# mFinn27/Template-Matching-and-Regression-MapReduce

Measured on AMD Instinct MI355X. Metric: images/sec (whole node) match+regress+NMS; % HBM/MFMA roofline at 1/2/4/8 GPU, higher is better.
Workload: dtype fp32; 1 GPU; config B: 64x SAM feats 256x64x64 (->128x128), 3 exemplars, templates 3x3-15x15, fp32, cls 0.1, IoU 0.5; config=B, images_per_gpu=64, exemplars=3, parallelism=dp1, decoder=split, decoder_precision=fp32

## Files before the change

### template-matching-and-regression-mapreduce_amd/csrc/conv_split.hip

```cpp
#include <algorithm>
#include <type_traits>

#include "tmr_common.h"

namespace {

typedef _Float16 h8 __attribute__((ext_vector_type(8)));
typedef __bf16 b8 __attribute__((ext_vector_type(8)));
typedef float f32x4 __attribute__((ext_vector_type(4)));
typedef __bf16 b4 __attribute__((ext_vector_type(4)));
typedef __attribute__((address_space(3))) void *lds_ptr_t;


constexpr int BM = 128;
constexpr int TH = 16;
constexpr int TW = 32;
constexpr int LDS_KB = 160;
constexpr int PXG = 8, NG = 4;
constexpr int NWAVES = 8;
constexpr int NTHREADS = NWAVES * 64;
constexpr int WNS = (NWAVES == 8 || TH == 8) ? 2 : 1;
static_assert(TH == 4 * NWAVES / WNS, "a wave owns 4 output rows");
constexpr int NIN = 8 / WNS;
constexpr int ACCW = NIN * 8 * 64 * 4;
// ... 332 lines not shown
                }
        }
    } else {
#pragma unroll
        for (int in = 0; in < NIN; ++in)
#pragma unroll
            for (int jp = 0; jp < 8; ++jp)
#pragma unroll
                for (int r = 0; r < 4; ++r) acc[in][jp][r] = 0.0f;
    }

    const int aoff = kg * WPL + (wn * 64 + l16) * 16;
    const int boff = kg * HPL + (wpix * 4 * HC + l16) * 16;

    auto ipt_of = [](bool lo_) { return lo_ ? 8 : G::NPLW * 2; };
#pragma unroll
    for (int m = 0; m < MPW; ++m) halo_dma1(0, m);
#pragma unroll
    for (int g0 = 0; g0 < D; ++g0) {
        const bool lo0 = HALVES == 2 && ((g0 / SPC) & 1);
        const int nt0 = min(TPS, T - (g0 % SPC) * TPS) * ipt_of(lo0) / NWAVES;
#pragma unroll
        for (int m = 0; m < nt0; ++m) w_dma1(g0, ipt_of(lo0), m);
    }
    asm volatile("s_waitcnt vmcnt(0)" ::: "memory");
    __builtin_amdgcn_s_barrier();
    for (int c = 0; c < NC; ++c) {
        auto half_chunk = [&](auto part_c) {
            constexpr int part = decltype(part_c)::value;
            constexpr bool lo = part == 1;
            const int hc = c * HALVES + part;
            const char *hl = Hs + (hc & 1) * HB;
            auto step = [&](auto sg_c) {
                constexpr int sg = decltype(sg_c)::value;
                constexpr bool L3 = G::LO3;
                constexpr int TPSx = L3 ? G::tps(part) : TPS;
                const int g = L3 ? c * G::SPCC + (part ? SPC : 0) + sg : hc * SPC + sg;
                constexpr bool lastx = sg + 1 >= G::spc(part);
                constexpr int pn = lastx ? 1 - part : part, sgn = lastx ? 0 : sg + 1;
                constexpr int nh = L3 ? G::nhp(part, sg) : G::nh(sg);
                constexpr bool loD = L3 ? pn == 1 : G::lo_of(sg + D, part, HALVES);
                constexpr int nw = L3 ? G::ntapp(pn, sgn) * G::ipt(pn == 1) / NWAVES : G::nw(sg, part, HALVES);
                constexpr int NSLOT = nh + nw;
                auto dma_slot = [&](int k) {
                    if constexpr (L3) {
                        if (k < nh)
                            halo_dma1(hc + 1, sg * G::qh(part) + k);
                        else
                            w_dma3(lastx && part == 1 ? c + 1 : c, pn, sgn, ipt_of(loD), k - nh);
                    } else {
                        if (k < nh)
                            halo_dma1(hc + 1, sg * Q + k);
                        else
                            w_dma1(g + D, ipt_of(loD), k - nh);
                    }
                };
                const char *wl = Ws + (g % NWB) * WB;
                constexpr int NA = (HALVES == 2 && !lo) ? 2 * NIN : NIN;
                constexpr int DB = NA >= 8 ? 1 : 2;
                constexpr int APG = NA >= 8 ? NA / 8 : 1;
                constexpr int NB = DB + 1;
                constexpr int ntap = L3 ? G::ntapp(part, sg) : (T - sg * TPS < TPS ? T - sg * TPS : TPS);
                constexpr int WB1x = L3 ? G::wb1(part) : WB1;
                auto afrag = [&](int tl, int i) -> V {
                    return *reinterpret_cast<const V *>(wl + tl * WB1x + (i / NIN) * 4 * WPL + aoff +
                                                        (i % NIN) * 256);
                };
                auto bfrag = [&](int tap, int jp) -> V {
                    const int ky = tap / KS, kx = tap % KS;
                    return *reinterpret_cast<const V *>(
                        hl + boff + (((jp >> 1) + ky) * HC + kx + (jp & 1) * 16) * 16);
                };
                V aw[2][NA];
                V bx[NB];
#pragma unroll
                for (int i = 0; i < NA; ++i) aw[0][i] = afrag(0, i);
#pragma unroll
                for (int d = 0; d < DB; ++d) bx[d] = bfrag(sg * TPSx, d);
                __builtin_amdgcn_sched_group_barrier(0x100, NA + DB, 0);
#pragma unroll
                for (int tl = 0; tl < TPSx; ++tl) {
                    if (tl >= ntap) break;
                    const int tap = sg * TPSx + tl;
                    const bool more = tl + 1 < ntap;
#pragma unroll
                    for (int jp = 0; jp < 8; ++jp) {
                        const int q = tl * 8 + jp, qn = q + DB;
                        const bool rb = jp + DB < 8 || more;
                        if (rb) bx[qn % NB] = jp + DB < 8 ? bfrag(tap, jp + DB) : bfrag(tap + 1, jp + DB - 8);
                        const int na = (more && jp * APG < NA) ? APG : 0;
#pragma unroll
                        for (int j = 0; j < APG; ++j)
                            if (j < na) aw[(tl + 1) & 1][jp * APG + j] = afrag(tl + 1, jp * APG + j);
                        const int k = q - 1;
                        const bool dm = k >= 0 && k < NSLOT;
                        if (dm) dma_slot(k);
                        const V b = bx[q % NB];
#pragma unroll
                        for (int i = 0; i < NA; ++i)
                            acc[i % NIN][jp] = mma(aw[tl & 1][i], b, acc[i % NIN][jp]);
                        const int nr = (rb ? 1 : 0) + na;
                        if (nr == 3)
                            __builtin_amdgcn_sched_group_barrier(0x100, 3, 0);
                        else if (nr == 2)
                            __builtin_amdgcn_sched_group_barrier(0x100, 2, 0);
                        else if (nr == 1)
                            __builtin_amdgcn_sched_group_barrier(0x100, 1, 0);
                        if (dm) __builtin_amdgcn_sched_group_barrier(0x020, 1, 0);
                        __builtin_amdgcn_sched_group_barrier(0x008, NA, 0);
                    }
                }
#pragma unroll
                for (int k = 0; k < 16; ++k)
                    if (k >= ntap * 8 - 1 && k < NSLOT) dma_slot(k);
                __builtin_amdgcn_sched_barrier(0);
                if constexpr (D == 1)
                    asm volatile("s_waitcnt vmcnt(0)" ::: "memory");
                else
                    wait_vmcnt(G::allowed(sg, part, HALVES));
                __builtin_amdgcn_s_barrier();
            };
            [&]<int... SG>(std::integer_sequence<int, SG...>) {
                (step(std::integral_constant<int, SG>{}), ...);
            }(std::make_integer_sequence<int, G::LO3 ? G::spc(part) : SPC>{});
        };
        half_chunk(std::integral_constant<int, 0>{});
        if constexpr (HALVES == 2) half_chunk(std::integral_constant<int, 1>{});
    }
    asm volatile("s_waitcnt vmcnt(0)" ::: "memory");

    const float inv = 1.0f / sxw;
    if (EPI == 0 && (a.flags & TMR_SPLIT_TILED_OUT) && (a.flags & TMR_SPLIT_OUT_BF16)) {
        b4 *o = reinterpret_cast<b4 *>(a.out) + ((((size_t)u * a.NT + nt) * a.MT + mt) * NWAVES + wave) * ACCW / 4 +
                lane;
#pragma unroll
        for (int in = 0; in < NIN; ++in)
#pragma unroll
            for (int jp = 0; jp < 8; ++jp)
                __builtin_nontemporal_store(__builtin_convertvector(acc[in][jp] * inv, b4), o + (in * 8 + jp) * 64);
        return;
    }
    if (EPI == 0 && (a.flags & TMR_SPLIT_TILED_OUT)) {
        f32x4 *o = reinterpret_cast<f32x4 *>(
                       a.out + ((((size_t)u * a.NT + nt) * a.MT + mt) * NWAVES + wave) * ACCW) +
                   lane;
#pragma unroll
        for (int in = 0; in < NIN; ++in)
#pragma unroll
            for (int jp = 0; jp < 8; ++jp) {
                __builtin_nontemporal_store(acc[in][jp] * inv, o + (in * 8 + jp) * 64);
            }
        return;
    }
    float *red = reinterpret_cast<float *>(lds);
    float *sb = red + 4 * 8 * NHEAD * 16;
    float *shw = sb + BM;
    if (tid < BM) {
        const int n = nt * BM + tid;
        sb[tid] = n < a.N ? a.bias[n] : 0.0f;
    }
    if (EPI == 1)
        for (int e = tid; e < BM * NHEAD; e += NTHREADS) shw[e] = a.headw[(size_t)nt * BM * NHEAD + e];
    __syncthreads();
    if constexpr (EPI == 0) {
        float invp[8];
#pragma unroll
        for (int jp = 0; jp < 8; ++jp) {
            invp[jp] = inv;
            const int y = ty0 + wpix * 4 + (jp >> 1), x = tx0 + (jp & 1) * 16 + l16;
            if (PR::SCALED && (a.flags & TMR_SPLIT_XMAX_PER_PIXEL) && y < a.H && x < a.W)
                invp[jp] = 1.0f / (split_scale(a.xmax + ((size_t)u * a.H + y) * a.W + x) * split_scale(a.wmax));
        }
#pragma unroll
        for (int in = 0; in < NIN; ++in)
#pragma unroll
            for (int r = 0; r < 4; ++r) {
                const int nl = wn * 64 + in * 16 + 4 * kg + r;
                const int n = nt * BM + nl;
                const bool nin = n < a.N;
                const float bn = sb[nl];
#pragma unroll
                for (int jp = 0; jp < 8; ++jp) {
                    const int y = ty0 + wpix * 4 + (jp >> 1), x = tx0 + (jp & 1) * 16 + l16;
                    float v = acc[in][jp][r] * invp[jp] + bn;
                    if (a.leaky) v = v >= 0.0f ? v : v * 0.01f;
                    if (nin && y < a.H && x < a.W) a.out[((size_t)u * a.N + n) * HW + (size_t)y * a.W + x] = v;
                }
            }
        return;
    }
    f2 hs2[4][NHEAD];
#pragma unroll
    for (int q = 0; q < 4; ++q)
#pragma unroll
        for (int k = 0; k < NHEAD; ++k) hs2[q][k] = (f2){0.0f, 0.0f};
    const f2 inv2 = {inv, inv};
#pragma unroll
    for (int in = 0; in < NIN; ++in)
#pragma unroll
        for (int r = 0; r < 4; ++r) {
            const int nl = wn * 64 + in * 16 + 4 * kg + r;
            const f2 bn2 = {sb[nl], sb[nl]};
            f2 hw2[NHEAD];
#pragma unroll
            for (int k = 0; k < NHEAD; ++k) hw2[k] = (f2){shw[nl * NHEAD + k], shw[nl * NHEAD + k]};
#pragma unroll
            for (int q = 0; q < 4; ++q)
                head_fma(head_act((f2){acc[in][2 * q][r], acc[in][2 * q + 1][r]}, inv2, bn2, a.leaky), hw2, hs2[q]);
            __builtin_amdgcn_sched_barrier(0);
        }
    float X[40];
#pragma unroll
    for (int q = 0; q < 4; ++q)
#pragma unroll
        for (int k = 0; k < NHEAD; ++k) {
            X[2 * (5 * q + k)] = hs2[q][k].x;
            X[2 * (5 * q + k) + 1] = hs2[q][k].y;
        }
    float Y[20], Z[10];
#pragma unroll
    for (int m = 0; m < 20; ++m) {
        const auto s = __builtin_amdgcn_permlane16_swap(__float_as_uint(X[2 * m]), __float_as_uint(X[2 * m + 1]),
                                                         false, false);
        Y[m] = __uint_as_float(s[0]) + __uint_as_float(s[1]);
    }
#pragma unroll
    for (int p = 0; p < 10; ++p) {
        const auto s = __builtin_amdgcn_permlane32_swap(__float_as_uint(Y[2 * p]), __float_as_uint(Y[2 * p + 1]),
                                                         false, false);
        Z[p] = __uint_as_float(s[0]) + __uint_as_float(s[1]);
    }
    __syncthreads();
    if (WNS == 2 && wn == 1) {
#pragma unroll
        for (int p = 0; p < 10; ++p) red[((wpix * 10 + p) * 4 + kg) * 16 + l16] = Z[p];
    }
    __syncthreads();
    if (wn == 0) {
#pragma unroll
        for (int p = 0; p < 10; ++p) {
            const int j = 4 * p + kg, m = j >> 1, q = m / NHEAD, k = m - q * NHEAD;
            const int jp = 2 * q + (j & 1);
            const int y = ty0 + wpix * 4 + (jp >> 1), x = tx0 + (jp & 1) * 16 + l16;
            const float v = Z[p] + (WNS == 2 ? red[((wpix * 10 + p) * 4 + kg) * 16 + l16] : 0.0f);
            if (y < a.H && x < a.W) a.partials[(((size_t)nt * NHEAD + k) * a.U + u) * HW + (size_t)y * a.W + x] = v;
        }
    }
}

template <int KS, int PREC, int EPI>
int launch_split(SArgs a, hipStream_t s) {
    constexpr size_t lds = Geo<KS, PREC>::LDS;
    static_assert(lds <= 160 * 1024, "LDS");
    static_assert((4 * 8 * NHEAD * 16 + BM * (NHEAD + 1)) * 4 <= lds, "epilogue scratch");
    auto kern = split_conv_kernel<KS, PREC, EPI>;
    if (tmr_set_max_lds((const void *)kern, lds) !=
        hipSuccess)
        return TMR_E_HIP;
    const int64_t blocks = (int64_t)a.NTW * a.MT * a.U;
    if (blocks <= 0) return TMR_OK;
    TMR_REQUIRE(blocks < (1ll << 31));
    hipLaunchKernelGGL(kern, dim3((unsigned)blocks), dim3(NTHREADS), lds, s, a);
    TMR_CHECK_LAUNCH();
    return TMR_OK;
}

template <int KS, int EPI>
int dispatch_prec(int prec, const SArgs &a, hipStream_t s) {
    switch (prec) {
        case TMR_PREC_F16X3: return launch_split<KS, TMR_PREC_F16X3, EPI>(a, s);
        case TMR_PREC_BF16: return launch_split<KS, TMR_PREC_BF16, EPI>(a, s);
        case TMR_PREC_F16: return launch_split<KS, TMR_PREC_F16, EPI>(a, s);
        default: return TMR_E_INVALID;
    }
}

template <int EPI>
int dispatch_ks(int ks, int prec, const SArgs &a, hipStream_t s) {
    switch (ks) {
        case 1: return dispatch_prec<1, EPI>(prec, a, s);
        case 3: return dispatch_prec<3, EPI>(prec, a, s);
        case 5: return dispatch_prec<5, EPI>(prec, a, s);
        case 7: return dispatch_prec<7, EPI>(prec, a, s);
        default: return TMR_E_INVALID;
    }
}

constexpr int PT = TMR_POINTS_TILE;
constexpr int PP = 2 * PT;
constexpr int PCG = PP / 16;
constexpr int PTW = NWAVES / WNS;
static_assert(PT == 64 && 4 * PP == NTHREADS, "points block: one store lane per head and point");
static_assert(WNS == 2 && NWAVES == 2 * P, "points block: a wave per 64-channel half; gathers dealt by (piece, half)");

struct PArgs {
    SArgs s;
    const float *head_bias;
    const float *box;
    const int32_t *tiles;
    int ntiles;
    float *b;
};

template <int KS, int PREC>
__global__ __launch_bounds__(NTHREADS) void split_points_kernel(PArgs pa) {
    typedef Prec<PREC> PR;
    typedef typename PR::V V;
    constexpr int T = KS * KS, HALVES = PR::HALVES, WREC = PR::WREC;
    constexpr int NF = NIN;
    constexpr int NS = HALVES == 2 ? 3 * T : T;
    const SArgs &a = pa.s;
    constexpr int BB = T * P * PP * 16;
    extern __shared__ __attribute__((aligned(16))) char plds[];
    char *Bs = plds;
    float(*red)[4][PP] = reinterpret_cast<float(*)[4][PP]>(plds + 2 * BB);
    float(*xch)[4][PP] = reinterpret_cast<float(*)[4][PP]>(plds + BB);
    static_assert(PTW * 4 * PP * sizeof(float) <= BB, "the odd waves' sums fit a B buffer");

    const int tid = threadIdx.x;
    const int lane = tid & 63;
    const int wave = __builtin_amdgcn_readfirstlane(tid >> 6);
    const int wh = wave & 1, wt = wave >> 1;
    const int l16 = lane & 15, kg = lane >> 4;
    const int HW = a.H * a.W;
    int tu[2], tfirst[2], tcnt[2], timg[2];
    float sxw[2];
#pragma unroll
    for (int hh = 0; hh < 2; ++hh) {
        const int64_t ti = 2 * (int64_t)blockIdx.x + hh;
        const bool have = ti < pa.ntiles;
        const int32_t *tl = pa.tiles + 3 * (have ? ti : ti - hh);
        tu[hh] = min(max(tl[0], 0), a.U - 1);
        tfirst[hh] = min(max(tl[1], 0), HW - 1);
        tcnt[hh] = have ? min(max(tl[2], 0), PT) : 0;
        timg[hh] = a.unit_image ? a.unit_image[tu[hh]] : tu[hh];
        sxw[hh] = split_sxw<PREC>(a, tu[hh]);
    }
    const int NC = a.NC0 + a.NC1;
    auto pixel = [&](int u, int first, int cnt, int p) {
        const int *pixi = reinterpret_cast<const int *>(pa.box) + 4 * (size_t)u * HW;
        return min(max(pixi[4 * (size_t)min(first + (p < cnt ? p : 0), HW - 1)], 0), HW - 1);
    };
    const int gu = wh ? tu[1] : tu[0], gfirst = wh ? tfirst[1] : tfirst[0], gcnt = wh ? tcnt[1] : tcnt[0];
    const int gimg = wh ? timg[1] : timg[0];

    const uint32_t cstride = (uint32_t)a.Hp * a.Wp * XREC;
    const int h0 = a.NC0 * HALVES, h1 = a.NC1 * HALVES;
    const __amdgpu_buffer_rsrc_t xr0 = __builtin_amdgcn_make_buffer_rsrc(
        (void *)(h0 ? a.x0 + (size_t)gimg * h0 * cstride : a.x1), (short)0, h0 * cstride, 0x00020000);
    const __amdgpu_buffer_rsrc_t xr1 = __builtin_amdgcn_make_buffer_rsrc(
        (void *)(h1 ? a.x1 + (size_t)gu * h1 * cstride : a.x0), (short)0, h1 * cstride, 0x00020000);
    const uint32_t tapstride = (uint32_t)NC * a.Npad * WREC;
    const __amdgpu_buffer_rsrc_t wr = __builtin_amdgcn_make_buffer_rsrc(
        (void *)a.wp, (short)0, T * tapstride, 0x00020000);
    uint32_t goff[KS];
#pragma unroll
    for (int i = 0; i < KS; ++i) {
        const int g = 64 * i + lane;
        const int pix = pixel(gu, gfirst, gcnt, g / KS), y = pix / a.W;
        goff[i] = (uint32_t)(y * a.Wp + (pix - y * a.W) + g % KS) * 16;
    }
    const uint32_t qstride = (uint32_t)a.Hp * a.Wp * 16;
    auto gather = [&](int hc) {
        const bool s0 = hc < h0;
        const uint32_t hs_ = (uint32_t)(s0 ? hc : hc - h0) * cstride + wt * qstride;
#pragma unroll
        for (int ky = 0; ky < KS; ++ky)
#pragma unroll
            for (int i = 0; i < KS; ++i)
                buffer_lds16(s0 ? xr0 : xr1,
                             (lds_ptr_t)(Bs + (hc & 1) * BB + (((ky * P + wt) * PP + wh * PT) * KS + 64 * i) * 16), goff[i],
                             hs_ + (uint32_t)(ky * a.Wp) * 16);
    };
    const int bfo = kg * (PP * KS * 16) + l16 * (KS * 16);
    auto bfrag = [&](int hc, int tap, int j) -> V {
        return *reinterpret_cast<const V *>(Bs + (hc & 1) * BB + (tap / KS) * (P * PP * KS * 16) + bfo +
                                            j * (16 * KS * 16) + (tap % KS) * 16);
    };

    const int npass = a.NTW > PTW ? 2 : 1;
    for (int pass = 0; pass < npass; ++pass) {
        const int wtile = pass * PTW + wt;
        const bool active = wtile < a.NTW;
        const int nt = a.NT0 + (active ? wtile : 0);
        const uint32_t aoff = (uint32_t)kg * a.Npad * 16 + ((uint32_t)nt * BM + wh * (BM / 2) + l16) * 16;
        gather(0);

        f32x4 acc[NF][PCG];
        if (a.acc_init) {
            const bool i16 = a.flags & TMR_SPLIT_INIT_BF16;
#pragma unroll
            for (int j = 0; j < PCG; ++j) {
                constexpr int HJ = PCG / 2;
                const int hh = j / HJ;
                const int pix = pixel(tu[hh], tfirst[hh], tcnt[hh], (j % HJ) * 16 + l16);
                const int py = pix / a.W, px = pix - py * a.W;
                const float sx = sxw[hh];
                const int islab = (a.flags & TMR_SPLIT_INIT_BCAST) ? 0 : timg[hh];
                const int mt = (py / TH) * a.TXN + px / TW;
                const int wpix = (py % TH) >> 2, jp = ((py & 3) << 1) | ((px % TW) >> 4);
                const size_t g4 = (((((size_t)islab * a.NT + nt) * a.MT + mt) * NWAVES + wpix * WNS + wh) * ACCW) / 4 +
                                  jp * 64 + kg * 16 + (px & 15);
                if (i16) {
                    const b4 *ai = reinterpret_cast<const b4 *>(a.acc_init) + g4;
#pragma unroll
                    for (int f = 0; f < NF; ++f)
                        acc[f][j] = __builtin_convertvector(ai[f * 8 * 64], f32x4) * sx;
                } else {
                    const f32x4 *ai = reinterpret_cast<const f32x4 *>(a.acc_init) + g4;
#pragma unroll
                    for (int f = 0; f < NF; ++f)
                        acc[f][j] = ai[f * 8 * 64] * sx;
                }
            }
        } else {
#pragma unroll
            for (int f = 0; f < NF; ++f)
#pragma unroll
                for (int j = 0; j < PCG; ++j) acc[f][j] = (f32x4){0.0f, 0.0f, 0.0f, 0.0f};
        }

        auto st_part = [](int s) { return HALVES == 2 && s >= 2 * T ? 1 : 0; };
        auto st_tap = [](int s) { return HALVES == 2 ? (s >= 2 * T ? s - 2 * T : s / 2) : s; };
        auto st_term = [](int s) { return HALVES == 2 && s < 2 * T ? s & 1 : 0; };
        auto st_newb = [](int s) { return !(HALVES == 2 && s < 2 * T && (s & 1)); };
        auto st_first = [](int s) { return s == 0 || (HALVES == 2 && s == 2 * T); };
        auto st_last = [](int s) { return s == NS - 1 || (HALVES == 2 && s == 2 * T - 1); };
        constexpr int AR = 3;
        static_assert(NS % AR == 0 && NS >= AR, "weight ring");
        V ar[AR][NF];
        auto load_stage = [&](int c, int s) {
            if (s >= NS) {
                s -= NS;
                c = c + 1 < NC ? c + 1 : c;
            }
            const uint32_t as = (uint32_t)st_tap(s) * tapstride + (uint32_t)c * a.Npad * WREC +
                                (uint32_t)st_term(s) * 4 * a.Npad * 16;
#pragma unroll
            for (int f = 0; f < NF; ++f) ar[s % AR][f] = buffer_load16<V>(wr, aoff + f * 256, as);
        };
#pragma unroll
        for (int s = 0; s < AR - 1; ++s) load_stage(0, s);
        asm volatile("s_waitcnt vmcnt(0)" ::: "memory");
        __syncthreads();
        V bc[PCG];
        const int NHC = NC * HALVES;
        for (int c = 0; c < NC; ++c) {
#pragma unroll
            for (int s = 0; s < NS; ++s) {
                const int hc = c * HALVES + st_part(s);
                load_stage(c, s + AR - 1);
                if (st_first(s)) {
                    if (hc + 1 < NHC) gather(hc + 1);
#pragma unroll
                    for (int j = 0; j < PCG; ++j) bc[j] = bfrag(hc, st_tap(s), j);
                }
                const bool nextb = s + 1 < NS && st_newb(s + 1) && !st_first(s + 1);
                __builtin_amdgcn_sched_barrier(0);
#pragma unroll
                for (int j = 0; j < PCG; ++j) {
#pragma unroll
                    for (int f = 0; f < NF; ++f) acc[f][j] = mma(ar[s % AR][f], bc[j], acc[f][j]);
                    if (nextb) {
                        bc[j] = bfrag(hc, st_tap(s + 1), j);
                        __builtin_amdgcn_sched_barrier(0);
                    }
                }
                __builtin_amdgcn_sched_barrier(0);
                if (st_last(s)) {
                    static_assert((AR - 1) * NF == 8 && T > AR - 1, "the counted wait below");
                    asm volatile("s_waitcnt vmcnt(8)" ::: "memory");
                    __syncthreads();
                }
            }
        }

        f2 hs[PCG / 2][NHEAD];
#pragma unroll
        for (int q = 0; q < PCG / 2; ++q)
#pragma unroll
            for (int k = 0; k < NHEAD; ++k) hs[q][k] = (f2){0.0f, 0.0f};
#pragma unroll
        for (int f = 0; f < NF; ++f)
#pragma unroll
            for (int r = 0; r < 4; ++r) {
                const int n = nt * BM + wh * (BM / 2) + f * 16 + 4 * kg + r;
                const float bv = n < a.N ? a.bias[n] : 0.0f;
                const f2 bn2 = {bv, bv};
                f2 hw2[NHEAD];
#pragma unroll
                for (int k = 0; k < NHEAD; ++k) {
                    const float h = a.headw[(size_t)n * NHEAD + k];
                    hw2[k] = (f2){h, h};
                }
#pragma unroll
                for (int q = 0; q < PCG / 2; ++q) {
                    const float inv = 1.0f / sxw[q / (PCG / 4)];
                    head_fma(head_act((f2){acc[f][2 * q][r], acc[f][2 * q + 1][r]}, (f2){inv, inv}, bn2, a.leaky), hw2,
                             hs[q]);
                }
            }
        float z[PCG / 2][4][2];
#pragma unroll
        for (int q = 0; q < PCG / 2; ++q)
#pragma unroll
            for (int k = 0; k < 4; ++k)
#pragma unroll
                for (int e = 0; e < 2; ++e) {
                    const float x = hs[q][k][e];
                    const float y = x + __shfl_xor(x, 16);
                    z[q][k][e] = y + __shfl_xor(y, 32);
                }
        if (wh == 1 && kg == 0 && active) {
#pragma unroll
            for (int q = 0; q < PCG / 2; ++q)
#pragma unroll
                for (int k = 0; k < 4; ++k)
#pragma unroll
                    for (int e = 0; e < 2; ++e) xch[wt][k][(2 * q + e) * 16 + l16] = z[q][k][e];
        }
        __syncthreads();
        if (wh == 0 && kg == 0 && active) {
#pragma unroll
            for (int q = 0; q < PCG / 2; ++q)
#pragma unroll
                for (int k = 0; k < 4; ++k)
#pragma unroll
                    for (int e = 0; e < 2; ++e) {
                        const int p = (2 * q + e) * 16 + l16;
                        red[wtile][k][p] = z[q][k][e] + xch[wt][k][p];
                    }
        }
    }
    __syncthreads();
    {
        const int k = tid / PP, p = tid % PP, pl = p % PT;
        if (pl < gcnt) {
            const int pix = pixel(gu, gfirst, gcnt, pl);
            float s = 0.0f;
            for (int t = 0; t < a.NTW; ++t) s += red[t][k][p];
            pa.b[((size_t)gu * 4 + k) * HW + pix] = s + pa.head_bias[k];
        }
    }
}

template <int PREC>
int launch_points(const PArgs &pa, int ntiles, hipStream_t s) {
    constexpr size_t lds = 2 * 9 * P * PP * 16 + NWAVES * 4 * PP * sizeof(float);
    static_assert(lds <= LDS_KB * 1024, "LDS");
    auto kern = split_points_kernel<3, PREC>;
    if (tmr_set_max_lds((const void *)kern, lds) != hipSuccess) return TMR_E_HIP;
    hipLaunchKernelGGL(kern, dim3((unsigned)((ntiles + 1) / 2)), dim3(NTHREADS), lds, s, pa);
    TMR_CHECK_LAUNCH();
    return TMR_OK;
}

inline int prec_halves(int prec) { return prec == TMR_PREC_F16X3 ? 2 : 1; }
inline int prec_wrec(int prec) { return prec == TMR_PREC_F16X3 ? 128 : 64; }
inline bool prec_ok(int prec) {
    return prec == TMR_PREC_F16X3 || prec == TMR_PREC_BF16 || prec == TMR_PREC_F16;
}
inline bool ks_ok(int ks) { return ks == 1 || ks == 3 || ks == 5 || ks == 7; }
inline bool tile_window(int flags, int NT, int &first, int &count) {
    first = (flags >> TMR_SPLIT_TILE_FIRST_SHIFT) & 0xff;
    count = (flags >> TMR_SPLIT_TILE_COUNT_SHIFT) & 0x7f;
    if (count == 0) {
        if (first != 0) return false;
        count = NT;
    }
    return first + count <= NT;
}
inline int pad_h(int H, int ks) { return (int)tmr_cdiv(H, TH) * TH + ks - 1; }
inline int pad_w(int W, int ks) { return (int)tmr_cdiv(W, TW) * TW + ks - 1; }

__device__ __forceinline__ void absmax_commit(float m, unsigned *out) {
    __shared__ float red[4];
    for (int o = 32; o > 0; o >>= 1) m = fmaxf(m, __shfl_xor(m, o));
    if ((threadIdx.x & 63) == 0) red[threadIdx.x >> 6] = m;
    __syncthreads();
    if (threadIdx.x == 0) atomicMax(out, __float_as_uint(fmaxf(fmaxf(red[0], red[1]), fmaxf(red[2], red[3]))));
}

__global__ __launch_bounds__(256) void absmax_rows_kernel(const float *__restrict__ x, int64_t n, int vec,
                                                          unsigned *__restrict__ out) {
    const float *xr = x + (size_t)blockIdx.y * n;
    float m = 0.0f;
    const int64_t step = (int64_t)gridDim.x * blockDim.x;
    if (vec) {
        const float4 *x4 = reinterpret_cast<const float4 *>(xr);
        for (int64_t i = (int64_t)blockIdx.x * blockDim.x + threadIdx.x; i < n / 4; i += step) {
            const float4 v = x4[i];
            m = fmaxf(m, fmaxf(fmaxf(fabsf(v.x), fabsf(v.y)), fmaxf(fabsf(v.z), fabsf(v.w))));
        }
    } else {
        for (int64_t i = (int64_t)blockIdx.x * blockDim.x + threadIdx.x; i < n; i += step)
            m = fmaxf(m, fabsf(xr[i]));
    }
    absmax_commit(m, out + blockIdx.y);
}

constexpr int PA_PIX = 64, PA_GRP = 8;
__global__ __launch_bounds__(PA_PIX * PA_GRP) void pixel_absmax_kernel(const float *__restrict__ x, int S, int C,
                                                                       int64_t HW, float *__restrict__ out) {
    __shared__ float part[PA_GRP][PA_PIX];
    const int lane = threadIdx.x & (PA_PIX - 1), grp = threadIdx.x / PA_PIX;
    const int64_t i = (int64_t)blockIdx.x * PA_PIX + lane;
    float m = 0.0f;
    if (i < (int64_t)S * HW) {
        const int64_t s = i / HW, p = i - s * HW;
        const float *xp = x + (size_t)s * C * HW + p;
#pragma unroll 8
        for (int c = grp; c < C; c += PA_GRP) m = fmaxf(m, fabsf(xp[(size_t)c * HW]));
    }
    part[grp][lane] = m;
    __syncthreads();
    if (grp == 0 && i < (int64_t)S * HW) {
#pragma unroll
        for (int g = 1; g < PA_GRP; ++g) m = fmaxf(m, part[g][lane]);
        out[i] = m;
    }
}

__global__ __launch_bounds__(256) void scale_merge_kernel(const float *__restrict__ img_max,
                                                          const float *__restrict__ unit_max,
                                                          const int32_t *__restrict__ unit_image, int U,
                                                          float *__restrict__ out_img,
                                                          float *__restrict__ out_unit) {
    __shared__ float red[4];
    const int b = blockIdx.x;
    float m = 0.0f;
    for (int u = threadIdx.x; u < U; u += blockDim.x)
        if (unit_image[u] == b) m = fmaxf(m, unit_max[u]);
    for (int o = 32; o > 0; o >>= 1) m = fmaxf(m, __shfl_xor(m, o));
    if ((threadIdx.x & 63) == 0) red[threadIdx.x >> 6] = m;
    __syncthreads();
    m = fmaxf(fmaxf(red[0], red[1]), fmaxf(red[2], red[3]));
    if (img_max) m = fmaxf(m, img_max[b]);
    if (threadIdx.x == 0 && out_img) out_img[b] = m;
    for (int u = threadIdx.x; u < U; u += blockDim.x)
        if (unit_image[u] == b) out_unit[u] = m;
}

template <int PREC, int MODE>
__global__ void xpack_kernel(const float *__restrict__ x, int S, int Cin, int Hin, int Win, int ups,
                             int ones, int H, int W, int NCc, int Hp, int Wp, int pad,
                             const float *__restrict__ xmax, int xms,
                             typename Prec<PREC>::V *__restrict__ out) {
    constexpr int HALVES = Prec<PREC>::HALVES;
    const int64_t total = (int64_t)S * NCc * Hp * Wp;
    const int64_t i = (int64_t)blockIdx.x * blockDim.x + threadIdx.x;
    if (i >= total) return;
    const int xp = (int)(i % Wp);
    int64_t r = i / Wp;
    const int yp = (int)(r % Hp);
    r /= Hp;
    const int c = (int)(r % NCc);
    const int s = (int)(r / NCc);
    const int y = yp - pad, xx = xp - pad;
    const bool in = y >= 0 && y < H && xx >= 0 && xx < W;
    const float *xm = !xmax ? nullptr
                      : xms == 2 ? (in ? xmax + ((size_t)s * H + y) * W + xx : nullptr)
                                 : xmax + (size_t)s * xms;
    const float sc = Prec<PREC>::SCALED ? split_scale(xm) : 1.0f;
    float v[CCH];
#pragma unroll
    for (int k = 0; k < CCH; ++k) {
        const int ch = c * CCH + k;
        float val = 0.0f;
        if (in) {
            if (MODE == 0) {
                if (ch < Cin) val = x[(((size_t)s * Cin + ch) * H + y) * W + xx];
            } else if (ch < Cin) {
                const float *pl = x + ((size_t)s * Cin + ch) * Hin * Win;
                val = ups ? up_value(pl, Hin, Win, y, xx) : pl[(size_t)y * Win + xx];
            } else if (ones && ch == Cin) {
                val = 1.0f;
            }
        }
        v[k] = val;
    }
    typename Prec<PREC>::V hi[P], lo[P];
    split_record<PREC>(v, sc, hi, lo);
    const size_t plane = (size_t)Hp * Wp;
    typename Prec<PREC>::V *o = out + ((size_t)s * NCc + c) * HALVES * P * plane + (size_t)yp * Wp + xp;
#pragma unroll
    for (int q = 0; q < P; ++q) o[q * plane] = hi[q];
    if (HALVES == 2) {
#pragma unroll
        for (int q = 0; q < P; ++q) o[(P + q) * plane] = lo[q];
    }
}

constexpr int XSEG = 128;
constexpr int XPACK16_RPB = 4;
template <int PREC, typename IN = float, int RPB = 1>
__global__ __launch_bounds__(256) void xpack4_kernel(const IN *__restrict__ x, int S, int Cin, int H, int W,
                                                     int NCc, int Hp, int Wp, int pad, int64_t nseg,
                                                     int64_t nbord, const float *__restrict__ xmax, int xms,
                                                     typename Prec<PREC>::V *__restrict__ out) {
    constexpr int HALVES = Prec<PREC>::HALVES;
    typedef typename Prec<PREC>::V V;
    typedef typename Prec<PREC>::E E;
    constexpr int VE = 16 / sizeof(IN);
    constexpr int LPR = CCH * XSEG / VE;
    typedef IN INV __attribute__((ext_vector_type(VE)));
    static_assert(RPB * LPR % 256 == 0 && RPB * XSEG * P % 256 == 0 && XSEG % VE == 0, "xpack4 tiling");
    __shared__ __attribute__((aligned(16))) IN tile[RPB][CCH][XSEG];
    const size_t plane = (size_t)Hp * Wp;
    const int t = threadIdx.x;
    if ((int64_t)blockIdx.x < nseg) {
        const int nsx = (W + XSEG - 1) / XSEG, nyg = (H + RPB - 1) / RPB;
        int64_t r = blockIdx.x;
        const int sx = (int)(r % nsx);
        r /= nsx;
        const int y0 = (int)(r % nyg) * RPB;
        r /= nyg;
        const int c = (int)(r % NCc);
        const int s = (int)(r / NCc);
        const int x0 = sx * XSEG, nx = min(XSEG, W - x0);
        const IN *src = x + ((size_t)s * Cin + (size_t)c * CCH) * H * W + (size_t)y0 * W + x0;
#pragma unroll
        for (int k = 0; k < RPB * LPR / 256; ++k) {
            const int e = t + 256 * k, rr = e / LPR, ch = (e % LPR) / (XSEG / VE), xv = e % (XSEG / VE);
            INV v = {};
            if (VE * xv < nx && c * CCH + ch < Cin && y0 + rr < H)
                v = *reinterpret_cast<const INV *>(src + (size_t)ch * H * W + (size_t)rr * W + VE * xv);
            *reinterpret_cast<INV *>(&tile[rr][ch][VE * xv]) = v;
        }
        __syncthreads();
        const float sc = Prec<PREC>::SCALED ? split_scale(xmax ? xmax + (size_t)s * xms : nullptr) : 1.0f;
        V *o = out + ((size_t)s * NCc + c) * HALVES * P * plane + (size_t)(y0 + pad) * Wp + x0 + pad;
#pragma unroll
        for (int k = 0; k < RPB * XSEG * P / 256; ++k) {
            const int e = t + 256 * k, rr = e / (XSEG * P), q = (e % (XSEG * P)) / XSEG, px = e % XSEG;
            if (px < nx && y0 + rr < H) {
                V hi, lo;
#pragma unroll
                for (int m = 0; m < 8; ++m) {
                    const float xs = (float)tile[rr][q * 8 + m][px] * sc;
                    const E h = (E)xs;
                    hi[m] = h;
                    if (HALVES == 2) lo[m] = (E)(xs - (float)h);
                }
                o[q * plane + (size_t)rr * Wp + px] = hi;
                if (HALVES == 2) o[(P + q) * plane + (size_t)rr * Wp + px] = lo;
            }
        }
        return;
    }
    const int64_t b0 = ((int64_t)blockIdx.x - nseg) * 256 + t;
    if (b0 >= nbord * S * NCc) return;
    const int64_t sc_i = b0 / nbord;
    int64_t b = b0 - sc_i * nbord;
    const int64_t top = (int64_t)pad * Wp, bot = (int64_t)(Hp - H - pad) * Wp;
    int yp, xp;
    if (b < top) {
        yp = (int)(b / Wp), xp = (int)(b % Wp);
    } else if ((b -= top) < bot) {
        yp = H + pad + (int)(b / Wp), xp = (int)(b % Wp);
    } else {
        b -= bot;
        const int side = Wp - W, k = (int)(b % side);
        yp = pad + (int)(b / side), xp = k < pad ? k : W + k;
    }
    V *o = out + (size_t)sc_i * HALVES * P * plane + (size_t)yp * Wp + xp;
    const V z = {};
#pragma unroll
    for (int q = 0; q < HALVES * P; ++q) o[q * plane] = z;
}

__global__ void fold_proj_kernel(const float *__restrict__ wd, int N, int Cw, int Cp, int T,
                                 const float *__restrict__ pw, const float *__restrict__ pb,
                                 int Cin, float *__restrict__ out) {
    const int64_t total = (int64_t)N * (Cin + 1) * T;
    const int64_t i = (int64_t)blockIdx.x * blockDim.x + threadIdx.x;
    if (i >= total) return;
    const int t = (int)(i % T);
    const int64_t r = i / T;
    const int c = (int)(r % (Cin + 1));
    const int n = (int)(r / (Cin + 1));
    const float *w = wd + (size_t)n * Cw * T + t;
    double acc = 0.0;
    if (c < Cin) {
        for (int k = 0; k < Cp; ++k) acc += (double)w[(size_t)k * T] * (double)pw[(size_t)k * Cin + c];
    } else {
        for (int k = 0; k < Cp; ++k) acc += (double)w[(size_t)k * T] * (double)pb[k];
    }
    out[i] = (float)acc;
}

template <int PREC>
__global__ void wpack_kernel(const float *__restrict__ w, int N, int C0, int C1, int ks, int NC0,
                             int NC, int Npad, const float *__restrict__ wmax,
                             typename Prec<PREC>::V *__restrict__ out) {
    const int T = ks * ks;
    const int64_t total = (int64_t)T * NC * Npad;
    const int64_t i = (int64_t)blockIdx.x * blockDim.x + threadIdx.x;
    if (i >= total) return;
    const int n = (int)(i % Npad);
    int64_t r = i / Npad;
    const int c = (int)(r % NC);
    const int tap = (int)(r / NC);
    const int C = C0 + C1;
    const float sc = Prec<PREC>::SCALED ? split_scale(wmax) : 1.0f;
    float v[CCH];
#pragma unroll
    for (int k = 0; k < CCH; ++k) {
        int ch;
        bool ok;
        if (c < NC0) {
            ch = c * CCH + k;
            ok = ch < C0;
        } else {
            const int c1 = (c - NC0) * CCH + k;
            ch = C0 + c1;
            ok = c1 < C1;
        }
        v[k] = (ok && n < N) ? w[((size_t)n * C + ch) * T + tap] : 0.0f;
    }
    typename Prec<PREC>::V hi[P], lo[P];
    split_record_w<PREC>(v, sc, hi, lo);
    constexpr int NP = Prec<PREC>::WREC / 16;
    typename Prec<PREC>::V *o = out + ((size_t)tap * NC + c) * NP * Npad + n;
#pragma unroll
    for (int q = 0; q < P; ++q) o[(size_t)q * Npad] = hi[q];
    if (NP == 8) {
#pragma unroll
        for (int q = 0; q < P; ++q) o[(size_t)(P + q) * Npad] = lo[q];
    }
}

int split_common(const void *xp0, int C0, const int32_t *unit_image, const void *xp1, int C1, int U,
                 int H, int W, int ks, int prec, const void *wpack, const float *wmax,
                 const float *xmax, const float *bias, int N, int leaky, const float *acc_init,
                 float *out, const float *headw, float *partials, int epi, int flags, void *stream) {
    TMR_REQUIRE(prec_ok(prec) && ks_ok(ks));
    TMR_REQUIRE(wpack && bias && U > 0 && H > 0 && W > 0 && N > 0 && C0 >= 0 && C1 >= 0);
    TMR_REQUIRE(C0 + C1 > 0 && (C0 == 0 || xp0) && (C1 == 0 || xp1));
    TMR_REQUIRE(prec == TMR_PREC_BF16 || (wmax && xmax));
// ... 265 lines not shown
```

Before: 711.9 images/s.

## Cut register pressure in points kernel with sliding B window and scalarized tile state

The points kernel now keeps a rolling window of four B fragments instead of all column-group fragments, prefetching the next fragment as each MFMA column finishes. Per-tile scalars are forced uniform with readfirstlane, and the buffer descriptor is built per gather, with a zero-size descriptor for the out-of-range gather so the branch disappears. Bias and head-weight loads are double-buffered across row groups. Opaque asm copies of lane indices stop the compiler from hoisting address math into long-lived registers. The goal is fewer VGPRs and spills and better overlap of LDS reads with MFMA, at the cost of more LDS reads interleaved with the MFMAs and more scheduling barriers.

```diff
diff --git a/template-matching-and-regression-mapreduce_amd/csrc/conv_split.hip b/template-matching-and-regression-mapreduce_amd/csrc/conv_split.hip
--- a/template-matching-and-regression-mapreduce_amd/csrc/conv_split.hip
+++ b/template-matching-and-regression-mapreduce_amd/csrc/conv_split.hip
@@ -658,6 +658,11 @@
     float *b;
 };
 
+__device__ __forceinline__ int opaque(int v) {
+    asm volatile("" : "+v"(v));
+    return v;
+}
+
 template <int KS, int PREC>
 __global__ __launch_bounds__(NTHREADS) void split_points_kernel(PArgs pa) {
     typedef Prec<PREC> PR;
@@ -686,13 +691,15 @@
         const int64_t ti = 2 * (int64_t)blockIdx.x + hh;
         const bool have = ti < pa.ntiles;
         const int32_t *tl = pa.tiles + 3 * (have ? ti : ti - hh);
-        tu[hh] = min(max(tl[0], 0), a.U - 1);
-        tfirst[hh] = min(max(tl[1], 0), HW - 1);
-        tcnt[hh] = have ? min(max(tl[2], 0), PT) : 0;
-        timg[hh] = a.unit_image ? a.unit_image[tu[hh]] : tu[hh];
-        sxw[hh] = split_sxw<PREC>(a, tu[hh]);
+        tu[hh] = __builtin_amdgcn_readfirstlane(min(max(tl[0], 0), a.U - 1));
+        tfirst[hh] = __builtin_amdgcn_readfirstlane(min(max(tl[1], 0), HW - 1));
+        tcnt[hh] = __builtin_amdgcn_readfirstlane(have ? min(max(tl[2], 0), PT) : 0);
+        timg[hh] = __builtin_amdgcn_readfirstlane(a.unit_image ? a.unit_image[tu[hh]] : tu[hh]);
+        sxw[hh] = __builtin_bit_cast(
+            float, __builtin_amdgcn_readfirstlane(__builtin_bit_cast(int, split_sxw<PREC>(a, tu[hh]))));
     }
     const int NC = a.NC0 + a.NC1;
+    const int NHC = NC * HALVES;
     auto pixel = [&](int u, int first, int cnt, int p) {
         const int *pixi = reinterpret_cast<const int *>(pa.box) + 4 * (size_t)u * HW;
         return min(max(pixi[4 * (size_t)min(first + (p < cnt ? p : 0), HW - 1)], 0), HW - 1);
@@ -702,10 +709,9 @@
 
     const uint32_t cstride = (uint32_t)a.Hp * a.Wp * XREC;
     const int h0 = a.NC0 * HALVES, h1 = a.NC1 * HALVES;
-    const __amdgpu_buffer_rsrc_t xr0 = __builtin_amdgcn_make_buffer_rsrc(
-        (void *)(h0 ? a.x0 + (size_t)gimg * h0 * cstride : a.x1), (short)0, h0 * cstride, 0x00020000);
-    const __amdgpu_buffer_rsrc_t xr1 = __builtin_amdgcn_make_buffer_rsrc(
-        (void *)(h1 ? a.x1 + (size_t)gu * h1 * cstride : a.x0), (short)0, h1 * cstride, 0x00020000);
+    void *const xb0 = (void *)(h0 ? a.x0 + (size_t)gimg * h0 * cstride : a.x1);
+    void *const xb1 = (void *)(h1 ? a.x1 + (size_t)gu * h1 * cstride : a.x0);
+    const int xn0 = h0 * cstride, xn1 = h1 * cstride;
     const uint32_t tapstride = (uint32_t)NC * a.Npad * WREC;
     const __amdgpu_buffer_rsrc_t wr = __builtin_amdgcn_make_buffer_rsrc(
         (void *)a.wp, (short)0, T * tapstride, 0x00020000);
@@ -717,14 +723,18 @@
         goff[i] = (uint32_t)(y * a.Wp + (pix - y * a.W) + g % KS) * 16;
     }
     const uint32_t qstride = (uint32_t)a.Hp * a.Wp * 16;
-    auto gather = [&](int hc) {
-        const bool s0 = hc < h0;
-        const uint32_t hs_ = (uint32_t)(s0 ? hc : hc - h0) * cstride + wt * qstride;
+    auto gather = [&](int hc, int nhc) {
+        const bool live = hc < nhc;
+        const int hsrc = min(hc, nhc - 1);
+        const bool s0 = hsrc < h0;
+        const uint32_t hs_ = (uint32_t)(s0 ? hsrc : hsrc - h0) * cstride + wt * qstride;
+        const __amdgpu_buffer_rsrc_t xr = __builtin_amdgcn_make_buffer_rsrc(
+            s0 ? xb0 : xb1, (short)0, live ? (s0 ? xn0 : xn1) : 0, 0x00020000);
 #pragma unroll
         for (int ky = 0; ky < KS; ++ky)
 #pragma unroll
             for (int i = 0; i < KS; ++i)
-                buffer_lds16(s0 ? xr0 : xr1,
+                buffer_lds16(xr,
                              (lds_ptr_t)(Bs + (hc & 1) * BB + (((ky * P + wt) * PP + wh * PT) * KS + 64 * i) * 16), goff[i],
                              hs_ + (uint32_t)(ky * a.Wp) * 16);
     };
@@ -740,23 +750,24 @@
         const bool active = wtile < a.NTW;
         const int nt = a.NT0 + (active ? wtile : 0);
         const uint32_t aoff = (uint32_t)kg * a.Npad * 16 + ((uint32_t)nt * BM + wh * (BM / 2) + l16) * 16;
-        gather(0);
+        gather(0, NHC);
 
         f32x4 acc[NF][PCG];
         if (a.acc_init) {
             const bool i16 = a.flags & TMR_SPLIT_INIT_BF16;
+            const int pl16 = opaque(l16), pkg = opaque(kg);
 #pragma unroll
             for (int j = 0; j < PCG; ++j) {
                 constexpr int HJ = PCG / 2;
                 const int hh = j / HJ;
-                const int pix = pixel(tu[hh], tfirst[hh], tcnt[hh], (j % HJ) * 16 + l16);
+                const int pix = pixel(tu[hh], tfirst[hh], tcnt[hh], (j % HJ) * 16 + pl16);
                 const int py = pix / a.W, px = pix - py * a.W;
                 const float sx = sxw[hh];
                 const int islab = (a.flags & TMR_SPLIT_INIT_BCAST) ? 0 : timg[hh];
                 const int mt = (py / TH) * a.TXN + px / TW;
                 const int wpix = (py % TH) >> 2, jp = ((py & 3) << 1) | ((px % TW) >> 4);
                 const size_t g4 = (((((size_t)islab * a.NT + nt) * a.MT + mt) * NWAVES + wpix * WNS + wh) * ACCW) / 4 +
-                                  jp * 64 + kg * 16 + (px & 15);
+                                  jp * 64 + pkg * 16 + (px & 15);
                 if (i16) {
                     const b4 *ai = reinterpret_cast<const b4 *>(a.acc_init) + g4;
 #pragma unroll
@@ -779,7 +790,6 @@
         auto st_part = [](int s) { return HALVES == 2 && s >= 2 * T ? 1 : 0; };
         auto st_tap = [](int s) { return HALVES == 2 ? (s >= 2 * T ? s - 2 * T : s / 2) : s; };
         auto st_term = [](int s) { return HALVES == 2 && s < 2 * T ? s & 1 : 0; };
-        auto st_newb = [](int s) { return !(HALVES == 2 && s < 2 * T && (s & 1)); };
         auto st_first = [](int s) { return s == 0 || (HALVES == 2 && s == 2 * T); };
         auto st_last = [](int s) { return s == NS - 1 || (HALVES == 2 && s == 2 * T - 1); };
         constexpr int AR = 3;
@@ -799,28 +809,30 @@
         for (int s = 0; s < AR - 1; ++s) load_stage(0, s);
         asm volatile("s_waitcnt vmcnt(0)" ::: "memory");
         __syncthreads();
-        V bc[PCG];
-        const int NHC = NC * HALVES;
+        constexpr int BW = 4;
+        static_assert(PCG % BW == 0, "a column group's window slot is the same in every stage");
+        V bw[BW];
         for (int c = 0; c < NC; ++c) {
 #pragma unroll
             for (int s = 0; s < NS; ++s) {
                 const int hc = c * HALVES + st_part(s);
                 load_stage(c, s + AR - 1);
                 if (st_first(s)) {
-                    if (hc + 1 < NHC) gather(hc + 1);
-#pragma unroll
-                    for (int j = 0; j < PCG; ++j) bc[j] = bfrag(hc, st_tap(s), j);
+                    gather(hc + 1, NHC);
+#pragma unroll
+                    for (int j = 0; j < BW; ++j) bw[j] = bfrag(hc, st_tap(s), j);
                 }
-                const bool nextb = s + 1 < NS && st_newb(s + 1) && !st_first(s + 1);
+                const bool nexts = s + 1 < NS && !st_first(s + 1);
                 __builtin_amdgcn_sched_barrier(0);
 #pragma unroll
                 for (int j = 0; j < PCG; ++j) {
 #pragma unroll
-                    for (int f = 0; f < NF; ++f) acc[f][j] = mma(ar[s % AR][f], bc[j], acc[f][j]);
-                    if (nextb) {
-                        bc[j] = bfrag(hc, st_tap(s + 1), j);
-                        __builtin_amdgcn_sched_barrier(0);
-                    }
+                    for (int f = 0; f < NF; ++f) acc[f][j] = mma(ar[s % AR][f], bw[j % BW], acc[f][j]);
+                    if (j + BW < PCG)
+                        bw[j % BW] = bfrag(hc, st_tap(s), j + BW);
+                    else if (nexts)
+                        bw[j % BW] = bfrag(hc, st_tap(s + 1), j + BW - PCG);
+                    __builtin_amdgcn_sched_barrier(0);
                 }
                 __builtin_amdgcn_sched_barrier(0);
                 if (st_last(s)) {
@@ -836,17 +848,30 @@
         for (int q = 0; q < PCG / 2; ++q)
 #pragma unroll
             for (int k = 0; k < NHEAD; ++k) hs[q][k] = (f2){0.0f, 0.0f};
-#pragma unroll
-        for (int f = 0; f < NF; ++f)
+        const int ekg = opaque(kg), el16 = opaque(l16);
+        float bvs[2][4], hws[2][4][NHEAD];
+        auto load_rows = [&](int f) {
 #pragma unroll
             for (int r = 0; r < 4; ++r) {
-                const int n = nt * BM + wh * (BM / 2) + f * 16 + 4 * kg + r;
-                const float bv = n < a.N ? a.bias[n] : 0.0f;
+                const int n = nt * BM + wh * (BM / 2) + f * 16 + 4 * ekg + r;
+                bvs[f & 1][r] = n < a.N ? a.bias[n] : 0.0f;
+#pragma unroll
+                for (int k = 0; k < NHEAD; ++k) hws[f & 1][r][k] = a.headw[(size_t)n * NHEAD + k];
+            }
+        };
+        load_rows(0);
+#pragma unroll
+        for (int f = 0; f < NF; ++f) {
+            if (f + 1 < NF) load_rows(f + 1);
+            __builtin_amdgcn_sched_barrier(0);
+#pragma unroll
+            for (int r = 0; r < 4; ++r) {
+                const float bv = bvs[f & 1][r];
                 const f2 bn2 = {bv, bv};
                 f2 hw2[NHEAD];
 #pragma unroll
                 for (int k = 0; k < NHEAD; ++k) {
-                    const float h = a.headw[(size_t)n * NHEAD + k];
+                    const float h = hws[f & 1][r][k];
                     hw2[k] = (f2){h, h};
                 }
 #pragma unroll
@@ -856,6 +881,8 @@
                              hs[q]);
                 }
             }
+            __builtin_amdgcn_sched_barrier(0);
+        }
         float z[PCG / 2][4][2];
 #pragma unroll
         for (int q = 0; q < PCG / 2; ++q)
@@ -867,30 +894,31 @@
                     const float y = x + __shfl_xor(x, 16);
                     z[q][k][e] = y + __shfl_xor(y, 32);
                 }
-        if (wh == 1 && kg == 0 && active) {
+        if (wh == 1 && ekg == 0 && active) {
 #pragma unroll
             for (int q = 0; q < PCG / 2; ++q)
 #pragma unroll
                 for (int k = 0; k < 4; ++k)
 #pragma unroll
-                    for (int e = 0; e < 2; ++e) xch[wt][k][(2 * q + e) * 16 + l16] = z[q][k][e];
+                    for (int e = 0; e < 2; ++e) xch[wt][k][(2 * q + e) * 16 + el16] = z[q][k][e];
         }
         __syncthreads();
-        if (wh == 0 && kg == 0 && active) {
+        if (wh == 0 && ekg == 0 && active) {
 #pragma unroll
             for (int q = 0; q < PCG / 2; ++q)
 #pragma unroll
                 for (int k = 0; k < 4; ++k)
 #pragma unroll
                     for (int e = 0; e < 2; ++e) {
-                        const int p = (2 * q + e) * 16 + l16;
+                        const int p = (2 * q + e) * 16 + el16;
                         red[wtile][k][p] = z[q][k][e] + xch[wt][k][p];
                     }
         }
     }
     __syncthreads();
     {
-        const int k = tid / PP, p = tid % PP, pl = p % PT;
+        const int st = opaque((int)threadIdx.x);
+        const int k = st / PP, p = st % PP, pl = p % PT;
         if (pl < gcnt) {
             const int pix = pixel(gu, gfirst, gcnt, pl);
             float s = 0.0f;
```

Result: no change. 718.8 images/s, median of 6 (+1.0%).
